# hip-satomi/microbeSEG

Hardware: AMD Instinct MI355X
Metric: training crops/sec (256px) (higher is better)
Workload: dtype f32; 1 GPU; BASELINE configs[1]: DU-Net distance-map training step, filters [64, 1024], 256x256 crops, per-GPU batch 32, fp32, relu/bn, SmoothL1x2 + Adam(amsgrad); global_batch=32, parallelism=dp1, launch=eager

## Files before the change

### include/mseg_hip.h

```cpp
#ifndef MSEG_HIP_H
#define MSEG_HIP_H

#include <stddef.h>
#include <stdint.h>

#ifdef __cplusplus
extern "C" {
#endif

#define MSEG_OK 0
#define MSEG_EINVAL (-1)
#define MSEG_ELAUNCH (-2)
#define MSEG_EWORKSPACE (-3)

#define MSEG_ACT_NONE 0
#define MSEG_ACT_RELU 1
#define MSEG_ACT_LEAKY 2
#define MSEG_ACT_ELU 3
#define MSEG_ACT_MISH 4

#define MSEG_NORM_BN 0
#define MSEG_NORM_GN 1
#define MSEG_NORM_IN 2

// ... 4 lines not shown
  const float* scale;
  const float* shift;
  int32_t C;
  int32_t act;
  int32_t ss;
  int32_t dtype;
} MsegSrc;

#define MSEG_MODE_CONV 0
#define MSEG_MODE_TCONV 1
#define MSEG_EPI_PLAIN 0
#define MSEG_EPI_SCATTER2X2 1
#define MSEG_MORDER_LINEAR 0
#define MSEG_MORDER_PARITY 1
#define MSEG_PREC_F32 0
#define MSEG_PREC_BF16 1

typedef struct MsegIgemm {
  MsegSrc src[2];
  const float* w;
  const float* bias;
  float* dst0;
  float* dst1;
  int32_t nsrc, Cin, Kpad, Npad;
  int32_t NB, Hi, Wi, Ho, Wo;
  int32_t KH, KW, stride, pad, mode, morder;
  int32_t Ngemm, epi, split, ld0, ld1, acc0, acc1, Cq;
  int32_t precision;
  int32_t dst_dtype;
  void* ws;
  size_t ws_bytes;
  float* stats;
  int32_t stats_act;
  int32_t reserved0;
} MsegIgemm;

int mseg_igemm(const MsegIgemm* p, void* stream);

typedef struct MsegKernelInfo {
  char name[120];
  int32_t precision;
  int32_t launches;
  uint32_t grid, block;
  size_t workspace;
  int32_t stats_rows;
  int32_t reserved0;
} MsegKernelInfo;
int mseg_igemm_query(const MsegIgemm* p, MsegKernelInfo* info);
const char* mseg_last_kernel(void);
int mseg_f32_to_bf16(const float* src, uint16_t* dst, size_t n, void* stream);
size_t mseg_igemm_workspace_bytes(const MsegIgemm* p);
int mseg_igemm_set_persistent(int on);
int mseg_igemm_set_wide_tiles(int on);
int mseg_igemm_set_p8(int mode);

typedef struct MsegWgrad {
  MsegSrc P;
  MsegSrc Q[2];
  float* ws;
  float* dst;
  int32_t nq, Nch, Nch_store;
  int32_t NB, Hp, Wp, Hq, Wq;
  int32_t KH, KW, stride, pad;
  int32_t splits;
  int32_t phase;
  int32_t precision;
  int32_t reserved;
// ... 288 lines not shown
```

### microbeseg_amd/_lib.py

```python
import ctypes as C
import os
import pathlib

_HERE = pathlib.Path(__file__).resolve().parent
LIB_PATH = _HERE / "libmseg_hip.so"

ACT = {"none": 0, "relu": 1, "leakyrelu": 2, "elu": 3, "mish": 4}
NORM = {"bn": 0, "gn": 1, "in": 2}
MODE_CONV, MODE_TCONV = 0, 1
EPI_PLAIN, EPI_SCATTER2X2 = 0, 1
MORDER_LINEAR, MORDER_PARITY = 0, 1
ST_F32, ST_BF16 = 0, 1
PIX_U8, PIX_U16, PIX_I32, PIX_F32 = 0, 1, 2, 3
GATHER_RAW, GATHER_F32, GATHER_NORM, GATHER_I64 = 0, 1, 2, 3


class MsegLibraryError(RuntimeError):
    pass


class MsegSrc(C.Structure):
    _fields_ = [("ptr", C.c_void_p), ("scale", C.c_void_p), ("shift", C.c_void_p),
                ("C", C.c_int32), ("act", C.c_int32), ("ss", C.c_int32), ("dtype", C.c_int32)]


class MsegIgemm(C.Structure):
    _fields_ = [("src", MsegSrc * 2), ("w", C.c_void_p), ("bias", C.c_void_p), ("dst0", C.c_void_p),
                ("dst1", C.c_void_p),
                ("nsrc", C.c_int32), ("Cin", C.c_int32), ("Kpad", C.c_int32), ("Npad", C.c_int32),
                ("NB", C.c_int32), ("Hi", C.c_int32), ("Wi", C.c_int32), ("Ho", C.c_int32), ("Wo", C.c_int32),
                ("KH", C.c_int32), ("KW", C.c_int32), ("stride", C.c_int32), ("pad", C.c_int32),
                ("mode", C.c_int32), ("morder", C.c_int32),
                ("Ngemm", C.c_int32), ("epi", C.c_int32), ("split", C.c_int32), ("ld0", C.c_int32),
                ("ld1", C.c_int32), ("acc0", C.c_int32), ("acc1", C.c_int32), ("Cq", C.c_int32),
                ("precision", C.c_int32), ("dst_dtype", C.c_int32), ("ws", C.c_void_p), ("ws_bytes", C.c_size_t),
                ("stats", C.c_void_p), ("stats_act", C.c_int32), ("reserved0", C.c_int32)]


class MsegWgrad(C.Structure):
    _fields_ = [("P", MsegSrc), ("Q", MsegSrc * 2), ("ws", C.c_void_p), ("dst", C.c_void_p),
                ("nq", C.c_int32), ("Nch", C.c_int32), ("Nch_store", C.c_int32),
                ("NB", C.c_int32), ("Hp", C.c_int32), ("Wp", C.c_int32), ("Hq", C.c_int32), ("Wq", C.c_int32),
                ("KH", C.c_int32), ("KW", C.c_int32), ("stride", C.c_int32), ("pad", C.c_int32),
                ("splits", C.c_int32), ("phase", C.c_int32), ("precision", C.c_int32), ("reserved", C.c_int32)]


class MsegKernelInfo(C.Structure):
    _fields_ = [("name", C.c_char * 120), ("precision", C.c_int32), ("launches", C.c_int32), ("grid", C.c_uint32),
                ("block", C.c_uint32), ("workspace", C.c_size_t), ("stats_rows", C.c_int32), ("reserved0", C.c_int32)]


class MsegPackJob(C.Structure):
    _fields_ = [("src", C.c_void_p), ("dst", C.c_void_p), ("dst16", C.c_void_p),
                ("T", C.c_int32), ("R", C.c_int32), ("Rpad", C.c_int32), ("C", C.c_int32), ("Cpad", C.c_int32),
                ("st", C.c_int32), ("sr", C.c_int32), ("sc", C.c_int32),
                ("first_block", C.c_uint32), ("reserved", C.c_uint32)]


class MsegRangerJob(C.Structure):
    _fields_ = [("p", C.c_void_p), ("g", C.c_void_p), ("m", C.c_void_p), ("v", C.c_void_p), ("slow", C.c_void_p),
                ("n", C.c_uint64), ("rows", C.c_int32), ("step_lr", C.c_float), ("flags", C.c_uint32),
                ("reserved", C.c_uint32)]


class MsegTtaMember(C.Structure):
    _fields_ = [("ptr", C.c_void_p), ("frame_stride", C.c_int64), ("chan_stride", C.c_int64), ("row_stride", C.c_int64),
                ("pix_stride", C.c_int64), ("code", C.c_int32), ("reserved", C.c_int32)]


# ... 180 lines not shown
```

### microbeseg_amd/csrc/igemm.hip

```cpp
#include "common.h"
#include "igemm_common.h"
#include "bf16_affine.h"

int igemm_p8_try(const MsegIgemm& p, int tr, int m_fastest, int cus, hipStream_t st);

__device__ float g_ident_scale[MSEG_MAX_CH];
__device__ float g_ident_shift[MSEG_MAX_CH];
__global__ void init_ident_kernel() {
  for (int i = blockIdx.x * blockDim.x + threadIdx.x; i < MSEG_MAX_CH; i += gridDim.x * blockDim.x) {
    g_ident_scale[i] = 1.f;
    g_ident_shift[i] = 0.f;
  }
}


template <int BM, int BN, bool PER_SAMPLE, bool GENERIC_ACT>
__global__ __launch_bounds__(256) void igemm_kernel(const MsegIgemm p) {
  using Cfg = IgemmCfg<BM, BN>;
  constexpr int STAGE = (BM + BN) * LDS_STRIDE;
  __shared__ __attribute__((aligned(16))) float lds[2 * STAGE + 4];
  unsigned* tapmask_s = reinterpret_cast<unsigned*>(lds + 2 * STAGE);

  const int tid = threadIdx.x;
  const int lane = tid & 63;
  const int wave = tid >> 6;
  const int wm = wave / Cfg::WN, wn = wave % Cfg::WN;

  const int M = p.NB * p.Ho * p.Wo;
  const int ntiles_n = (p.Ngemm + BN - 1) / BN;
  const int lid = (int)xcd_logical_id(blockIdx.x, gridDim.x);
  const int tile_m = lid / ntiles_n;
  const int tile_n = lid - tile_m * ntiles_n;
  const int m0 = tile_m * BM, n0 = tile_n * BN;

  const int T = p.KH * p.KW;
  const int srow = tid >> 3;
  const int scol = tid & 7;
// ... 170 lines not shown
        for (int b = 0; b < Cfg::NB; ++b) {
          acc[a][b] = __builtin_amdgcn_mfma_f32_32x32x2f32(af[a].x, bf[b].x, acc[a][b], 0, 0, 0);
          acc[a][b] = __builtin_amdgcn_mfma_f32_32x32x2f32(af[a].y, bf[b].y, acc[a][b], 0, 0, 0);
          acc[a][b] = __builtin_amdgcn_mfma_f32_32x32x2f32(af[a].z, bf[b].z, acc[a][b], 0, 0, 0);
          acc[a][b] = __builtin_amdgcn_mfma_f32_32x32x2f32(af[a].w, bf[b].w, acc[a][b], 0, 0, 0);
        }
    }
    float* An = lds + (cur ^ 1) * STAGE;
#ifdef MSEG_ABLATE
    STAMP(s2);
    if (!(abl & 8)) commit(An, An + BM * LDS_STRIDE);
    STAMP(s3);
    if (!(abl & 2)) __syncthreads();
    STAMP(s4);
    t_issue += s1 - s0; t_mfma += s2 - s1; t_commit += s3 - s2; t_bar += s4 - s3;
#else
    commit(An, An + BM * LDS_STRIDE);
    __syncthreads();
#endif
    cur ^= 1;
    have = have_next;
  }

#ifdef MSEG_ABLATE
  if ((abl & 32) && p.dst1 && lane == 0 && blockIdx.x < 1024) {
    float* dbg = p.dst1 + ((size_t)blockIdx.x * 4 + wave) * 4;
    dbg[0] = (float)t_issue; dbg[1] = (float)t_mfma; dbg[2] = (float)t_commit; dbg[3] = (float)t_bar;
  }
#endif
  igemm_epilogue<IgemmCfg<BM, BN>>(acc, m0, n0, wm, wn, lane, M);
}

template <int BM, int BN, int TR, bool PER_SAMPLE, bool SB = false>
__global__ __launch_bounds__(256) void igemm_fast_kernel(const MsegIgemm p) {
  using Cfg = IgemmCfg<BM, BN>;
  constexpr int STAGE = (BM + BN) * LDS_STRIDE;
  __shared__ __attribute__((aligned(16))) float lds[(SB ? 1 : 2) * STAGE];

  const int tid = threadIdx.x;
  const int lane = tid & 63;
  const int wave = tid >> 6;
  const int wm = wave / Cfg::WN, wn = wave % Cfg::WN;
  const int M = p.NB * p.Ho * p.Wo;
  const int ntiles_n = (p.Ngemm + BN - 1) / BN;
  const int lid = (int)xcd_logical_id(blockIdx.x, gridDim.x);
  const int tile_m = lid / ntiles_n;
  const int tile_n = lid - tile_m * ntiles_n;
  const int m0 = tile_m * BM, n0 = tile_n * BN;
  const int T = p.KH * p.KW;
  const int srow = tid >> 3, scol = tid & 7;

  const TapGeom geom = make_geom(p);
  const long long tile_px = tile_base_pixel(p, geom, m0, M);
  int pix0[Cfg::AROWS];
  int rown[Cfg::AROWS];
  unsigned vmask[Cfg::AROWS];
#pragma unroll
  for (int i = 0; i < Cfg::AROWS; ++i) {
    const RowInfo r = decode_row(p, m0 + srow + 32 * i, M);
    const int iy0 = (r.oy * geom.sm - geom.dir * geom.pad) >> geom.sh, ix0 = (r.ox * geom.sm - geom.dir * geom.pad) >> geom.sh;
    pix0[i] = (int)(((long long)r.n * p.Hi + iy0) * p.Wi + ix0 - tile_px);
    rown[i] = r.n < 0 ? 0 : r.n;
    unsigned mk = 0u;
    for (int t = 0; t < T; ++t) {
      const int ky = t / p.KW, kx = t - ky * p.KW;
      int iy, ix;
      mk |= (unsigned)tap_coord(geom, r, ky, kx, iy, ix) << t;
    }
    vmask[i] = mk;
  }

  f32x16 acc[Cfg::MB][Cfg::NB];
#pragma unroll
  for (int a = 0; a < Cfg::MB; ++a)
#pragma unroll
    for (int b = 0; b < Cfg::NB; ++b)
#pragma unroll
      for (int r = 0; r < 16; ++r) acc[a][b][r] = 0.f;

  const int nchunks = (p.Cin + KC - 1) / KC;
  const int C0 = p.src[0].C;
  const unsigned OOB = 0x80000000u;

  const __amdgpu_buffer_rsrc_t rs0 = __builtin_amdgcn_make_buffer_rsrc(
      const_cast<float*>(p.src[0].ptr + tile_px * p.src[0].C), 0, 0x7ffffff0, 0x00020000);
  const __amdgpu_buffer_rsrc_t rs1 = __builtin_amdgcn_make_buffer_rsrc(
      const_cast<float*>((p.nsrc > 1 ? p.src[1].ptr : p.src[0].ptr) + tile_px * (p.nsrc > 1 ? p.src[1].C : p.src[0].C)), 0,
      0x7ffffff0, 0x00020000);
  const __amdgpu_buffer_rsrc_t rsw = __builtin_amdgcn_make_buffer_rsrc(const_cast<float*>(p.w), 0,
                                                                        T * p.Npad * p.Kpad * 4, 0x00020000);
  unsigned wvoff[Cfg::BROWS];
#pragma unroll
  for (int i = 0; i < Cfg::BROWS; ++i) wvoff[i] = ((unsigned)(n0 + srow + 32 * i) * (unsigned)p.Kpad + scol * 4u) * 4u;

  constexpr int NSC = (TR == 0) ? 1 : (PER_SAMPLE ? Cfg::AROWS : 1);
  float4 ra[Cfg::AROWS], rb[Cfg::BROWS], rsc[NSC], rsh[NSC];
  float rm[Cfg::AROWS];
  unsigned rowoff[Cfg::AROWS];
  int ract = 0;
  int cur_chunk = -1;
  bool cur_s1 = false;

  auto issue = [&](int chunk, int t, int ky, int kx) {
    const int c = chunk * KC + scol * 4;
    if (chunk != cur_chunk) {
      cur_chunk = chunk;
      cur_s1 = (p.nsrc > 1) && (chunk * KC >= C0);
      const unsigned sC4 = (unsigned)(cur_s1 ? p.src[1].C : p.src[0].C) * 4u;
      const unsigned cl4 = (unsigned)(cur_s1 ? c - C0 : c) * 4u;
#pragma unroll
      for (int i = 0; i < Cfg::AROWS; ++i) rowoff[i] = (unsigned)pix0[i] * sC4 + cl4;
      if (TR != 0) {
        const MsegSrc& s = cur_s1 ? p.src[1] : p.src[0];
        ract = s.act;
        const bool has_aff = s.scale != nullptr;
        const float* scp = has_aff ? s.scale : g_ident_scale;
        const float* shp = has_aff ? s.shift : g_ident_shift;
        const unsigned cl = (c < p.Cin) ? (cl4 >> 2) : 0u;
#pragma unroll
        for (int i = 0; i < NSC; ++i) {
          const size_t o = (size_t)(PER_SAMPLE ? rown[i] : 0) * (has_aff ? (unsigned)s.ss : 0u) + cl;
          rsc[i] = *reinterpret_cast<const float4*>(scp + o);
          rsh[i] = *reinterpret_cast<const float4*>(shp + o);
        }
      }
    }
    const unsigned cbit = (c < p.Cin) ? (1u << t) : 0u;
    const unsigned sC4 = (unsigned)(cur_s1 ? p.src[1].C : p.src[0].C) * 4u;
    const unsigned delta = (unsigned)(geom.dir * ((ky >> geom.sh) * p.Wi + (kx >> geom.sh))) * sC4;
#pragma unroll
    for (int i = 0; i < Cfg::AROWS; ++i) {
      const bool ok = (vmask[i] & cbit) != 0u;
      const unsigned vo = ok ? rowoff[i] + delta : OOB;
// ... 3 lines not shown
      if (TR != 0) rm[i] = ok ? 1.f : 0.f;
    }
    const unsigned wso = ((unsigned)t * (unsigned)p.Npad * (unsigned)p.Kpad + (unsigned)chunk * KC) * 4u;
#pragma unroll
    for (int i = 0; i < Cfg::BROWS; ++i) {
      const f32x4 v = __builtin_bit_cast(f32x4, __builtin_amdgcn_raw_buffer_load_b128(rsw, wvoff[i], wso, 0));
      rb[i] = make_float4(v[0], v[1], v[2], v[3]);
    }
  };

  auto commit = [&](float* As, float* Bs) {
    const float lo = (ract == MSEG_ACT_RELU) ? 0.f : -3.402823466e38f;
#pragma unroll
    for (int i = 0; i < Cfg::AROWS; ++i) {
      float4 v = ra[i];
      if (TR != 0) {
        if (TR == 2) {
          v = act_fwd4(v, ract);
        } else {
          v.x = clamp_lo(v.x, lo); v.y = clamp_lo(v.y, lo); v.z = clamp_lo(v.z, lo); v.w = clamp_lo(v.w, lo);
        }
        const float4 sc = rsc[PER_SAMPLE ? i : 0], sh = rsh[PER_SAMPLE ? i : 0];
        const float m = rm[i];
        v.x = (v.x * sc.x + sh.x) * m; v.y = (v.y * sc.y + sh.y) * m;
        v.z = (v.z * sc.z + sh.z) * m; v.w = (v.w * sc.w + sh.w) * m;
      }
      *reinterpret_cast<float4*>(As + (srow + 32 * i) * LDS_STRIDE + scol * 4) = v;
    }
#pragma unroll
    for (int i = 0; i < Cfg::BROWS; ++i)
      *reinterpret_cast<float4*>(Bs + (srow + 32 * i) * LDS_STRIDE + scol * 4) = rb[i];
  };

  unsigned long long taplist = 0ull, taplist_hi = 0ull;
  int nlive = 0;
  {
    int py = 0, px = 0;
    if (geom.sh) {
      const int cls = m0 / (M >> 2);
      py = cls >> 1; px = cls & 1;
    }
    for (int tt = 0; tt < T; ++tt) {
      const int ky_ = tt / p.KW, kx_ = tt - ky_ * p.KW;
      const bool live = (((py - geom.dir * (ky_ - geom.pad)) | (px - geom.dir * (kx_ - geom.pad))) & geom.sh) == 0;
      if (live) {
        const unsigned long long e = (unsigned long long)(tt | (ky_ << 4) | (kx_ << 6));
        if (nlive < 8) taplist |= e << (8 * nlive); else taplist_hi |= e << (8 * (nlive - 8));
        ++nlive;
      }
    }
  }
  auto tap_at = [&](int j) -> unsigned { return (unsigned)((j < 8 ? taplist >> (8 * j) : taplist_hi >> (8 * (j - 8))) & 0xffull); };
  int chunk = 0, j = 0;
  const int nsteps = nchunks * nlive;
  unsigned e0 = tap_at(0);
  issue(0, (int)(e0 & 15u), (int)((e0 >> 4) & 3u), (int)(e0 >> 6));
  commit(lds, lds + BM * LDS_STRIDE);
  __syncthreads();
  int cur = 0;
  const int li = lane & 31, lh = lane >> 5;
  for (int step = 0; step < nsteps; ++step) {
    if (step + 1 < nsteps) {
      j += 1;
      if (j >= nlive) { j = 0; ++chunk; }
    }
    e0 = tap_at(j);
    issue(chunk, (int)(e0 & 15u), (int)((e0 >> 4) & 3u), (int)(e0 >> 6));

    const float* As = lds + cur * STAGE;
    const float* Bs = As + BM * LDS_STRIDE;
#pragma unroll
    for (int kk = 0; kk < KC / 8; ++kk) {
      float4 af[Cfg::MB], bf[Cfg::NB];
#pragma unroll
      for (int a = 0; a < Cfg::MB; ++a)
        af[a] = *reinterpret_cast<const float4*>(As + (wm * Cfg::TM + a * 32 + li) * LDS_STRIDE + kk * 8 + lh * 4);
#pragma unroll
      for (int b = 0; b < Cfg::NB; ++b)
        bf[b] = *reinterpret_cast<const float4*>(Bs + (wn * Cfg::TN + b * 32 + li) * LDS_STRIDE + kk * 8 + lh * 4);
#pragma unroll
      for (int a = 0; a < Cfg::MB; ++a)
#pragma unroll
        for (int b = 0; b < Cfg::NB; ++b) {
          acc[a][b] = __builtin_amdgcn_mfma_f32_32x32x2f32(af[a].x, bf[b].x, acc[a][b], 0, 0, 0);
          acc[a][b] = __builtin_amdgcn_mfma_f32_32x32x2f32(af[a].y, bf[b].y, acc[a][b], 0, 0, 0);
          acc[a][b] = __builtin_amdgcn_mfma_f32_32x32x2f32(af[a].z, bf[b].z, acc[a][b], 0, 0, 0);
          acc[a][b] = __builtin_amdgcn_mfma_f32_32x32x2f32(af[a].w, bf[b].w, acc[a][b], 0, 0, 0);
        }
    }
    if (SB) {
      __syncthreads();
      commit(lds, lds + BM * LDS_STRIDE);
      __syncthreads();
    } else {
      float* An = lds + (cur ^ 1) * STAGE;
      commit(An, An + BM * LDS_STRIDE);
      __syncthreads();
      cur ^= 1;
    }
  }
  igemm_epilogue<IgemmCfg<BM, BN>>(acc, m0, n0, wm, wn, lane, M);
}

template <int BN>
struct HaloCfg {
  static constexpr int WN = (BN >= 128) ? 4 : 2;
  static constexpr int WM = 8 / WN;
  static constexpr int TM = 128 / WM, TN = BN / WN;
  static constexpr int MB = TM / 32, NB = TN / 32;
  static constexpr int BROWS = BN / 64;
};

template <int BN, int TR>
__global__ __launch_bounds__(512, 2) void igemm_halo_kernel(const MsegIgemm p, int tw_log2, int ksplit,
                                                            int chunks_per_split) {
  constexpr int BM = 128;
  using Cfg = HaloCfg<BN>;
  constexpr int HMAX = 264;
  constexpr int HL = (HMAX * 8 + 511) / 512;
  constexpr int ASTAGE = HMAX * LDS_STRIDE;
  constexpr int BSTAGE = BN * LDS_STRIDE;
  __shared__ __attribute__((aligned(16))) float lds[ASTAGE + 2 * BSTAGE];
  float* const Abuf = lds;
  float* const Bbuf = lds + ASTAGE;

  const int tid = threadIdx.x, lane = tid & 63, wave = tid >> 6;
  const int wm = wave / Cfg::WN, wn = wave % Cfg::WN;
  const int li = lane & 31, lh = lane >> 5;
  const int srow = tid >> 3, scol = tid & 7;
  const int TW = 1 << tw_log2, TH = BM >> tw_log2, HW2 = TW + 2;
  const int HROWS = (TH + 2) * HW2;
  const int H = p.Hi, W = p.Wi;
  const int M = p.NB * H * W;
  const int tiles_x = W >> tw_log2, tiles_y = (H + TH - 1) / TH;
// ... 1957 lines not shown
}

extern "C" size_t mseg_igemm_workspace_bytes(const MsegIgemm* pp) {
  if (!pp) return 0;
  const MsegIgemm& p = *pp;
  if (p.Ngemm <= 0 || p.Cin <= 0 || p.NB <= 0 || p.Hi <= 0 || p.Wi <= 0) return 0;
  int tw_log2 = 0, cps = 0;
  long long htiles = 0;
  if (!halo_geometry(p, p.Ngemm > 64 ? 128 : 64, &tw_log2, &htiles)) return 0;
  const int ks = halo_ksplit(htiles, (p.Cin + KC - 1) / KC, &cps);
  if (ks <= 1 || (p.Ngemm & 3)) return 0;
  return (size_t)ks * p.NB * p.Hi * p.Wi * p.Ngemm * sizeof(float);
}

static int igemm_dispatch(const MsegIgemm* pp, void* stream) {
  if (!pp) return MSEG_EINVAL;
  const MsegIgemm& p = *pp;
  if (p.nsrc < 1 || p.nsrc > 2) return MSEG_EINVAL;
  int csum = 0;
  for (int i = 0; i < p.nsrc; ++i) {
    if (check_src(p.src[i])) return MSEG_EINVAL;
    csum += p.src[i].C;
  }
  if (csum != p.Cin) return MSEG_EINVAL;
  if (!p.w || !p.dst0 || p.Kpad < p.Cin || (p.Kpad % KC) || p.Npad < p.Ngemm || (p.Npad % 128)) return MSEG_EINVAL;
  if (p.Cin > MSEG_MAX_CH) return MSEG_EINVAL;
  if (p.NB <= 0 || p.Hi <= 0 || p.Wi <= 0 || p.Ho <= 0 || p.Wo <= 0) return MSEG_EINVAL;
  if (p.KH <= 0 || p.KW <= 0 || p.KH * p.KW > 16) return MSEG_EINVAL;
  if (p.stride != 1 && p.stride != 2) return MSEG_EINVAL;
  if (p.mode != MSEG_MODE_CONV && p.mode != MSEG_MODE_TCONV) return MSEG_EINVAL;
  if (p.morder == MSEG_MORDER_PARITY && ((p.Ho | p.Wo) & 1)) return MSEG_EINVAL;
  if (p.Ngemm <= 0) return MSEG_EINVAL;
  if (p.precision != MSEG_PREC_F32 && p.precision != MSEG_PREC_BF16) return MSEG_EINVAL;
  if (p.dst_dtype != MSEG_ST_F32 && p.dst_dtype != MSEG_ST_BF16) return MSEG_EINVAL;
  const bool s16 = p.src[0].dtype == MSEG_ST_BF16;
  if (p.nsrc > 1 && p.src[1].dtype != p.src[0].dtype) return MSEG_EINVAL;
  if ((s16 || p.dst_dtype == MSEG_ST_BF16) && p.precision != MSEG_PREC_BF16) return MSEG_EINVAL;
  if (p.dst_dtype == MSEG_ST_BF16) {
    if ((p.Ngemm | p.ld0 | p.ld1 | p.Cq) & 1) return MSEG_EINVAL;
    if (p.split < p.Ngemm && (p.split & 1)) return MSEG_EINVAL;
    if (((uintptr_t)p.dst0 | (uintptr_t)p.dst1) & 3) return MSEG_EINVAL;
  }
  if (p.epi == MSEG_EPI_SCATTER2X2) {
    if (p.Cq <= 0 || p.Ngemm != 4 * p.Cq || p.morder != MSEG_MORDER_LINEAR) return MSEG_EINVAL;
  } else if (p.epi == MSEG_EPI_PLAIN) {
    if (p.split < p.Ngemm && !p.dst1) return MSEG_EINVAL;
  } else {
    return MSEG_EINVAL;
  }
  const long long M = (long long)p.NB * p.Ho * p.Wo;
  if (M <= 0 || M > 0x7fffffffLL) return MSEG_EINVAL;
  hipStream_t st = (hipStream_t)stream;
  mseg_dispatch_note(p.precision, 0);
  static bool ident_ready[64] = {false};
  int devid = 0;
  const bool dry = mseg_dispatch_dry() != 0;
  if (!dry) {
    if (hipGetDevice(&devid) != hipSuccess || devid < 0 || devid >= 64) return MSEG_ELAUNCH;
    if (!ident_ready[devid]) {
      MSEG_KL_AUX(init_ident_kernel, dim3(8), dim3(256), 0, st);
      MSEG_LAUNCH_CHECK();
      ident_ready[devid] = true;
    }
  }
  bool per_sample = false, generic = false;
  for (int i = 0; i < p.nsrc; ++i) {
// ... 139 lines not shown
      p.stride == 2 && p.pad == 0 && p.mode == MSEG_MODE_CONV && p.morder == MSEG_MORDER_LINEAR && p.nsrc == 1 &&
      p.Cin == 64 && p.Kpad == 64 && p.Ngemm == 128 && p.split >= p.Ngemm && !p.acc0 && !p.bias && (p.Wo % 32) == 0 &&
      p.Hi == 2 * p.Ho && p.Wi == 2 * p.Wo && (M % 64) == 0 && M / 64 >= 4 * (long long)c64p_workgroups()) {
    const dim3 pgrid((unsigned)c64p_workgroups());
    if (p.dst_dtype == MSEG_ST_BF16) MSEG_KL((igemm_ctd_bf16_kernel<true>), pgrid, dim3(512), 0, st, p, (int)(M / 64));
    else MSEG_KL((igemm_ctd_bf16_kernel<false>), pgrid, dim3(512), 0, st, p, (int)(M / 64));
    MSEG_LAUNCH_CHECK();
    return MSEG_OK;
  }
  if (p.precision == MSEG_PREC_BF16) {
    if (!fast) return MSEG_EINVAL;
    const int tr = plain ? 0 : (generic ? 2 : 1);
#define MSEG_FAST16_LAUNCH(BM_, BN_, TR_, PS_)                                                          \
  do {                                                                                                  \
    if (s16) MSEG_KL((igemm_fast_bf16_kernel<BM_, BN_, TR_, PS_, true>), grid, block, 0, st, p);   \
    else MSEG_KL((igemm_fast_bf16_kernel<BM_, BN_, TR_, PS_, false>), grid, block, 0, st, p);      \
  } while (0)
#define MSEG_FAST16_TILE(BM_, BN_)                                                        \
  do {                                                                                    \
    if (tr == 0) MSEG_FAST16_LAUNCH(BM_, BN_, 0, false);                                  \
    else if (tr == 1) { if (per_sample) MSEG_FAST16_LAUNCH(BM_, BN_, 1, true); else MSEG_FAST16_LAUNCH(BM_, BN_, 1, false); } \
    else { if (per_sample) MSEG_FAST16_LAUNCH(BM_, BN_, 2, true); else MSEG_FAST16_LAUNCH(BM_, BN_, 2, false); }              \
  } while (0)
    if (wide) MSEG_FAST16_TILE(128, 128); else MSEG_FAST16_TILE(128, 64);
#undef MSEG_FAST16_TILE
#undef MSEG_FAST16_LAUNCH
    MSEG_LAUNCH_CHECK();
    return MSEG_OK;
  }
  if (fast) {
    const int tr = plain ? 0 : (generic ? 2 : 1);
    const int live_taps = (p.mode == MSEG_MODE_TCONV && p.stride == 2) ? ((p.KH + 1) / 2) * ((p.KW + 1) / 2) : p.KH * p.KW;
    const bool short_k = ((p.Cin + KC - 1) / KC) * live_taps <= 8;
#define MSEG_FAST_LAUNCH(BM_, BN_, TR_, PS_)                                                              \
  do {                                                                                                    \
    if (short_k) MSEG_KL((igemm_fast_kernel<BM_, BN_, TR_, PS_, true>), grid, block, 0, st, p); \
    else MSEG_KL((igemm_fast_kernel<BM_, BN_, TR_, PS_, false>), grid, block, 0, st, p);        \
  } while (0)
#define MSEG_FAST_TILE(BM_, BN_)                                                          \
  do {                                                                                    \
    if (tr == 0) MSEG_FAST_LAUNCH(BM_, BN_, 0, false);                                    \
    else if (tr == 1) { if (per_sample) MSEG_FAST_LAUNCH(BM_, BN_, 1, true); else MSEG_FAST_LAUNCH(BM_, BN_, 1, false); } \
    else { if (per_sample) MSEG_FAST_LAUNCH(BM_, BN_, 2, true); else MSEG_FAST_LAUNCH(BM_, BN_, 2, false); }              \
  } while (0)
    if (wide) MSEG_FAST_TILE(128, 128); else MSEG_FAST_TILE(128, 64);
#undef MSEG_FAST_TILE
#undef MSEG_FAST_LAUNCH
    MSEG_LAUNCH_CHECK();
    return MSEG_OK;
  }
#define MSEG_IGEMM_LAUNCH(BM_, BN_, PS_, GA_) \
  MSEG_KL((igemm_kernel<BM_, BN_, PS_, GA_>), grid, block, 0, st, p)
  if (wide) {
    if (per_sample) { if (generic) MSEG_IGEMM_LAUNCH(128, 128, true, true); else MSEG_IGEMM_LAUNCH(128, 128, true, false); }
    else            { if (generic) MSEG_IGEMM_LAUNCH(128, 128, false, true); else MSEG_IGEMM_LAUNCH(128, 128, false, false); }
  } else {
    if (per_sample) { if (generic) MSEG_IGEMM_LAUNCH(128, 64, true, true); else MSEG_IGEMM_LAUNCH(128, 64, true, false); }
    else            { if (generic) MSEG_IGEMM_LAUNCH(128, 64, false, true); else MSEG_IGEMM_LAUNCH(128, 64, false, false); }
  }
#undef MSEG_IGEMM_LAUNCH
  MSEG_LAUNCH_CHECK();
  return MSEG_OK;
}

extern "C" int mseg_igemm(const MsegIgemm* pp, void* stream) {
  mseg_dispatch_begin(0);
  const int rc = igemm_dispatch(pp, stream);
  mseg_dispatch_end(nullptr);
  return rc;
}
// ... 100 lines not shown
```

Measured before the change: 243.8 crops/s.

## Make fp32 fast implicit-GEMM kernel persistent over multiple M tiles per workgroup

The fp32 fast implicit-GEMM kernel now loops over several M tiles per workgroup in a serpentine order, with the grid sized from CU count and occupancy. The next tile's row geometry and tap list are set up during the last K step of the current tile, and per-row geometry is staged through shared memory. Launch bounds now request two or three workgroups per CU. This aims to cut tail-wave waste and per-block setup cost, at the price of more register and LDS pressure and extra control flow in the main loop.

```diff
diff --git a/include/mseg_hip.h b/include/mseg_hip.h
--- a/include/mseg_hip.h
+++ b/include/mseg_hip.h
@@ -60,7 +60,7 @@
   size_t ws_bytes;
   float* stats;
   int32_t stats_act;
-  int32_t reserved0;
+  int32_t tiles_per_wg;
 } MsegIgemm;
 
 int mseg_igemm(const MsegIgemm* p, void* stream);
diff --git a/microbeseg_amd/_lib.py b/microbeseg_amd/_lib.py
--- a/microbeseg_amd/_lib.py
+++ b/microbeseg_amd/_lib.py
@@ -34,7 +34,7 @@
                 ("Ngemm", C.c_int32), ("epi", C.c_int32), ("split", C.c_int32), ("ld0", C.c_int32),
                 ("ld1", C.c_int32), ("acc0", C.c_int32), ("acc1", C.c_int32), ("Cq", C.c_int32),
                 ("precision", C.c_int32), ("dst_dtype", C.c_int32), ("ws", C.c_void_p), ("ws_bytes", C.c_size_t),
-                ("stats", C.c_void_p), ("stats_act", C.c_int32), ("reserved0", C.c_int32)]
+                ("stats", C.c_void_p), ("stats_act", C.c_int32), ("tiles_per_wg", C.c_int32)]
 
 
 class MsegWgrad(C.Structure):
diff --git a/microbeseg_amd/csrc/igemm.hip b/microbeseg_amd/csrc/igemm.hip
--- a/microbeseg_amd/csrc/igemm.hip
+++ b/microbeseg_amd/csrc/igemm.hip
@@ -239,10 +239,11 @@
 }
 
 template <int BM, int BN, int TR, bool PER_SAMPLE, bool SB = false>
-__global__ __launch_bounds__(256) void igemm_fast_kernel(const MsegIgemm p) {
+__global__ __launch_bounds__(256, (BN == 64 && SB && TR == 0) ? 3 : 2) void igemm_fast_kernel(const MsegIgemm p) {
   using Cfg = IgemmCfg<BM, BN>;
   constexpr int STAGE = (BM + BN) * LDS_STRIDE;
   __shared__ __attribute__((aligned(16))) float lds[(SB ? 1 : 2) * STAGE];
+  __shared__ int geo[3 * BM];
 
   const int tid = threadIdx.x;
   const int lane = tid & 63;
@@ -250,62 +251,93 @@
   const int wm = wave / Cfg::WN, wn = wave % Cfg::WN;
   const int M = p.NB * p.Ho * p.Wo;
   const int ntiles_n = (p.Ngemm + BN - 1) / BN;
+  const int mtiles = (M + BM - 1) / BM;
   const int lid = (int)xcd_logical_id(blockIdx.x, gridDim.x);
-  const int tile_m = lid / ntiles_n;
-  const int tile_n = lid - tile_m * ntiles_n;
-  const int m0 = tile_m * BM, n0 = tile_n * BN;
+  const int G = (int)gridDim.x / ntiles_n;
+  const int grp = lid / ntiles_n;
+  const int tile_n = lid - grp * ntiles_n;
+  const int n0 = tile_n * BN;
+  if (grp >= mtiles) return;
   const int T = p.KH * p.KW;
-  const int srow = tid >> 3, scol = tid & 7;
+  int srow = tid >> 3, scol = tid & 7;
 
   const TapGeom geom = make_geom(p);
-  const long long tile_px = tile_base_pixel(p, geom, m0, M);
   int pix0[Cfg::AROWS];
   int rown[Cfg::AROWS];
   unsigned vmask[Cfg::AROWS];
-#pragma unroll
-  for (int i = 0; i < Cfg::AROWS; ++i) {
-    const RowInfo r = decode_row(p, m0 + srow + 32 * i, M);
-    const int iy0 = (r.oy * geom.sm - geom.dir * geom.pad) >> geom.sh, ix0 = (r.ox * geom.sm - geom.dir * geom.pad) >> geom.sh;
-    pix0[i] = (int)(((long long)r.n * p.Hi + iy0) * p.Wi + ix0 - tile_px);
-    rown[i] = r.n < 0 ? 0 : r.n;
-    unsigned mk = 0u;
-    for (int t = 0; t < T; ++t) {
-      const int ky = t / p.KW, kx = t - ky * p.KW;
-      int iy, ix;
-      mk |= (unsigned)tap_coord(geom, r, ky, kx, iy, ix) << t;
-    }
-    vmask[i] = mk;
-  }
+  __amdgpu_buffer_rsrc_t rs0, rs1;
+  unsigned long long taplist = 0ull, taplist_hi = 0ull;
+  int nlive = 0;
+  int cur_chunk = -1;
+
+  auto setup = [&](int m0) {
+    const long long tile_px = tile_base_pixel(p, geom, m0, M);
+#pragma unroll
+    for (int i = 0; i < Cfg::AROWS; ++i) {
+      const RowInfo r = decode_row(p, m0 + srow + 32 * i, M);
+      const int iy0 = (r.oy * geom.sm - geom.dir * geom.pad) >> geom.sh, ix0 = (r.ox * geom.sm - geom.dir * geom.pad) >> geom.sh;
+      pix0[i] = (int)(((long long)r.n * p.Hi + iy0) * p.Wi + ix0 - tile_px);
+      rown[i] = r.n < 0 ? 0 : r.n;
+      unsigned ym = 0u, xm = 0u;
+      for (int k = 0; k < p.KH; ++k) {
+        const int ty = r.oy * geom.sm + geom.dir * (k - geom.pad), iy = ty >> geom.sh;
+        ym |= (unsigned)(((ty & geom.sh) == 0) & (iy >= 0) & (iy < geom.Hi)) << k;
+      }
+      for (int k = 0; k < p.KW; ++k) {
+        const int tx = r.ox * geom.sm + geom.dir * (k - geom.pad), ix = tx >> geom.sh;
+        xm |= (unsigned)(((tx & geom.sh) == 0) & (ix >= 0) & (ix < geom.Wi)) << k;
+      }
+      if (r.n < 0) ym = 0u;
+      unsigned mk = 0u;
+      for (int ky = 0; ky < p.KH; ++ky) mk |= (((ym >> ky) & 1u) ? xm : 0u) << (ky * p.KW);
+      vmask[i] = mk;
+      const int gr = srow + 32 * i;
+      geo[gr] = pix0[i]; geo[BM + gr] = (int)mk; geo[2 * BM + gr] = rown[i];
+    }
+    rs0 = __builtin_amdgcn_make_buffer_rsrc(const_cast<float*>(p.src[0].ptr + tile_px * p.src[0].C), 0, 0x7ffffff0,
+                                            0x00020000);
+    rs1 = __builtin_amdgcn_make_buffer_rsrc(
+        const_cast<float*>((p.nsrc > 1 ? p.src[1].ptr : p.src[0].ptr) + tile_px * (p.nsrc > 1 ? p.src[1].C : p.src[0].C)), 0,
+        0x7ffffff0, 0x00020000);
+    int py = 0, px = 0;
+    if (geom.sh) {
+      const int cls = m0 / (M >> 2);
+      py = cls >> 1; px = cls & 1;
+    }
+    taplist = 0ull; taplist_hi = 0ull; nlive = 0;
+    int tt = 0;
+    for (int ky_ = 0; ky_ < p.KH; ++ky_)
+      for (int kx_ = 0; kx_ < p.KW; ++kx_, ++tt) {
+        const bool live = (((py - geom.dir * (ky_ - geom.pad)) | (px - geom.dir * (kx_ - geom.pad))) & geom.sh) == 0;
+        if (live) {
+          const unsigned long long e = (unsigned long long)(tt | (ky_ << 4) | (kx_ << 6));
+          if (nlive < 8) taplist |= e << (8 * nlive); else taplist_hi |= e << (8 * (nlive - 8));
+          ++nlive;
+        }
+      }
+    cur_chunk = -1;
+  };
 
   f32x16 acc[Cfg::MB][Cfg::NB];
-#pragma unroll
-  for (int a = 0; a < Cfg::MB; ++a)
-#pragma unroll
-    for (int b = 0; b < Cfg::NB; ++b)
-#pragma unroll
-      for (int r = 0; r < 16; ++r) acc[a][b][r] = 0.f;
 
   const int nchunks = (p.Cin + KC - 1) / KC;
   const int C0 = p.src[0].C;
   const unsigned OOB = 0x80000000u;
 
-  const __amdgpu_buffer_rsrc_t rs0 = __builtin_amdgcn_make_buffer_rsrc(
-      const_cast<float*>(p.src[0].ptr + tile_px * p.src[0].C), 0, 0x7ffffff0, 0x00020000);
-  const __amdgpu_buffer_rsrc_t rs1 = __builtin_amdgcn_make_buffer_rsrc(
-      const_cast<float*>((p.nsrc > 1 ? p.src[1].ptr : p.src[0].ptr) + tile_px * (p.nsrc > 1 ? p.src[1].C : p.src[0].C)), 0,
-      0x7ffffff0, 0x00020000);
   const __amdgpu_buffer_rsrc_t rsw = __builtin_amdgcn_make_buffer_rsrc(const_cast<float*>(p.w), 0,
                                                                         T * p.Npad * p.Kpad * 4, 0x00020000);
   unsigned wvoff[Cfg::BROWS];
-#pragma unroll
-  for (int i = 0; i < Cfg::BROWS; ++i) wvoff[i] = ((unsigned)(n0 + srow + 32 * i) * (unsigned)p.Kpad + scol * 4u) * 4u;
+  auto set_wvoff = [&]() {
+#pragma unroll
+    for (int i = 0; i < Cfg::BROWS; ++i) wvoff[i] = ((unsigned)(n0 + srow + 32 * i) * (unsigned)p.Kpad + scol * 4u) * 4u;
+  };
+  set_wvoff();
 
   constexpr int NSC = (TR == 0) ? 1 : (PER_SAMPLE ? Cfg::AROWS : 1);
   float4 ra[Cfg::AROWS], rb[Cfg::BROWS], rsc[NSC], rsh[NSC];
   float rm[Cfg::AROWS];
   unsigned rowoff[Cfg::AROWS];
   int ract = 0;
-  int cur_chunk = -1;
   bool cur_s1 = false;
 
   auto issue = [&](int chunk, int t, int ky, int kx) {
@@ -375,74 +407,89 @@
       *reinterpret_cast<float4*>(Bs + (srow + 32 * i) * LDS_STRIDE + scol * 4) = rb[i];
   };
 
-  unsigned long long taplist = 0ull, taplist_hi = 0ull;
-  int nlive = 0;
-  {
-    int py = 0, px = 0;
-    if (geom.sh) {
-      const int cls = m0 / (M >> 2);
-      py = cls >> 1; px = cls & 1;
-    }
-    for (int tt = 0; tt < T; ++tt) {
-      const int ky_ = tt / p.KW, kx_ = tt - ky_ * p.KW;
-      const bool live = (((py - geom.dir * (ky_ - geom.pad)) | (px - geom.dir * (kx_ - geom.pad))) & geom.sh) == 0;
-      if (live) {
-        const unsigned long long e = (unsigned long long)(tt | (ky_ << 4) | (kx_ << 6));
-        if (nlive < 8) taplist |= e << (8 * nlive); else taplist_hi |= e << (8 * (nlive - 8));
-        ++nlive;
-      }
-    }
-  }
   auto tap_at = [&](int j) -> unsigned { return (unsigned)((j < 8 ? taplist >> (8 * j) : taplist_hi >> (8 * (j - 8))) & 0xffull); };
+  int tile_m = grp, blk = 0;
+  setup(tile_m * BM);
   int chunk = 0, j = 0;
-  const int nsteps = nchunks * nlive;
+  int nsteps = nchunks * nlive;
   unsigned e0 = tap_at(0);
   issue(0, (int)(e0 & 15u), (int)((e0 >> 4) & 3u), (int)(e0 >> 6));
   commit(lds, lds + BM * LDS_STRIDE);
   __syncthreads();
   int cur = 0;
-  const int li = lane & 31, lh = lane >> 5;
-  for (int step = 0; step < nsteps; ++step) {
-    if (step + 1 < nsteps) {
-      j += 1;
-      if (j >= nlive) { j = 0; ++chunk; }
-    }
-    e0 = tap_at(j);
-    issue(chunk, (int)(e0 & 15u), (int)((e0 >> 4) & 3u), (int)(e0 >> 6));
-
-    const float* As = lds + cur * STAGE;
-    const float* Bs = As + BM * LDS_STRIDE;
-#pragma unroll
-    for (int kk = 0; kk < KC / 8; ++kk) {
-      float4 af[Cfg::MB], bf[Cfg::NB];
-#pragma unroll
-      for (int a = 0; a < Cfg::MB; ++a)
-        af[a] = *reinterpret_cast<const float4*>(As + (wm * Cfg::TM + a * 32 + li) * LDS_STRIDE + kk * 8 + lh * 4);
+  int li = lane & 31, lh = lane >> 5;
+  for (;;) {
+    const int m0 = tile_m * BM;
+    const int nblk = blk + 1;
+    const int next_m = nblk * G + ((nblk & 1) ? G - 1 - grp : grp);
+    const bool more = next_m < mtiles;
+    int nsteps_next = 0;
+#pragma unroll
+    for (int a = 0; a < Cfg::MB; ++a)
 #pragma unroll
       for (int b = 0; b < Cfg::NB; ++b)
-        bf[b] = *reinterpret_cast<const float4*>(Bs + (wn * Cfg::TN + b * 32 + li) * LDS_STRIDE + kk * 8 + lh * 4);
-#pragma unroll
-      for (int a = 0; a < Cfg::MB; ++a)
-#pragma unroll
-        for (int b = 0; b < Cfg::NB; ++b) {
-          acc[a][b] = __builtin_amdgcn_mfma_f32_32x32x2f32(af[a].x, bf[b].x, acc[a][b], 0, 0, 0);
-          acc[a][b] = __builtin_amdgcn_mfma_f32_32x32x2f32(af[a].y, bf[b].y, acc[a][b], 0, 0, 0);
-          acc[a][b] = __builtin_amdgcn_mfma_f32_32x32x2f32(af[a].z, bf[b].z, acc[a][b], 0, 0, 0);
-          acc[a][b] = __builtin_amdgcn_mfma_f32_32x32x2f32(af[a].w, bf[b].w, acc[a][b], 0, 0, 0);
-        }
-    }
-    if (SB) {
-      __syncthreads();
-      commit(lds, lds + BM * LDS_STRIDE);
-      __syncthreads();
-    } else {
-      float* An = lds + (cur ^ 1) * STAGE;
-      commit(An, An + BM * LDS_STRIDE);
-      __syncthreads();
-      cur ^= 1;
-    }
-  }
-  igemm_epilogue<IgemmCfg<BM, BN>>(acc, m0, n0, wm, wn, lane, M);
+#pragma unroll
+        for (int r = 0; r < 16; ++r) acc[a][b][r] = 0.f;
+    for (int step = 0; step < nsteps; ++step) {
+      if (step + 1 < nsteps) {
+        j += 1;
+        if (j >= nlive) { j = 0; ++chunk; }
+      } else if (more) {
+        setup(next_m * BM);
+        nsteps_next = nchunks * nlive;
+        chunk = 0; j = 0;
+      }
+      e0 = tap_at(j);
+      issue(chunk, (int)(e0 & 15u), (int)((e0 >> 4) & 3u), (int)(e0 >> 6));
+
+      const float* As = lds + cur * STAGE;
+      const float* Bs = As + BM * LDS_STRIDE;
+#pragma unroll
+      for (int kk = 0; kk < KC / 8; ++kk) {
+        float4 af[Cfg::MB], bf[Cfg::NB];
+#pragma unroll
+        for (int a = 0; a < Cfg::MB; ++a)
+          af[a] = *reinterpret_cast<const float4*>(As + (wm * Cfg::TM + a * 32 + li) * LDS_STRIDE + kk * 8 + lh * 4);
+#pragma unroll
+        for (int b = 0; b < Cfg::NB; ++b)
+          bf[b] = *reinterpret_cast<const float4*>(Bs + (wn * Cfg::TN + b * 32 + li) * LDS_STRIDE + kk * 8 + lh * 4);
+#pragma unroll
+        for (int a = 0; a < Cfg::MB; ++a)
+#pragma unroll
+          for (int b = 0; b < Cfg::NB; ++b) {
+            acc[a][b] = __builtin_amdgcn_mfma_f32_32x32x2f32(af[a].x, bf[b].x, acc[a][b], 0, 0, 0);
+            acc[a][b] = __builtin_amdgcn_mfma_f32_32x32x2f32(af[a].y, bf[b].y, acc[a][b], 0, 0, 0);
+            acc[a][b] = __builtin_amdgcn_mfma_f32_32x32x2f32(af[a].z, bf[b].z, acc[a][b], 0, 0, 0);
+            acc[a][b] = __builtin_amdgcn_mfma_f32_32x32x2f32(af[a].w, bf[b].w, acc[a][b], 0, 0, 0);
+          }
+      }
+      if (SB) {
+        __syncthreads();
+        commit(lds, lds + BM * LDS_STRIDE);
+        __syncthreads();
+      } else {
+        float* An = lds + (cur ^ 1) * STAGE;
+        commit(An, An + BM * LDS_STRIDE);
+        __syncthreads();
+        cur ^= 1;
+      }
+    }
+    igemm_epilogue<IgemmCfg<BM, BN>>(acc, m0, n0, wm, wn, lane, M);
+    if (!more) break;
+    tile_m = next_m;
+    blk = nblk;
+    int t_ = tid;
+    asm volatile("" : "+v"(t_));
+    srow = t_ >> 3; scol = t_ & 7; li = t_ & 31; lh = (t_ >> 5) & 1;
+#pragma unroll
+    for (int i = 0; i < Cfg::AROWS; ++i) {
+      const int gr = srow + 32 * i;
+      pix0[i] = geo[gr]; vmask[i] = (unsigned)geo[BM + gr]; rown[i] = geo[2 * BM + gr];
+    }
+    set_wvoff();
+    cur_chunk = -1;
+    nsteps = nsteps_next;
+  }
 }
 
 template <int BN>
@@ -2466,6 +2513,7 @@
   if (p.morder == MSEG_MORDER_PARITY && ((p.Ho | p.Wo) & 1)) return MSEG_EINVAL;
   if (p.Ngemm <= 0) return MSEG_EINVAL;
   if (p.precision != MSEG_PREC_F32 && p.precision != MSEG_PREC_BF16) return MSEG_EINVAL;
+  if (p.tiles_per_wg < 0 || p.tiles_per_wg > 64) return MSEG_EINVAL;
   if (p.dst_dtype != MSEG_ST_F32 && p.dst_dtype != MSEG_ST_BF16) return MSEG_EINVAL;
   const bool s16 = p.src[0].dtype == MSEG_ST_BF16;
   if (p.nsrc > 1 && p.src[1].dtype != p.src[0].dtype) return MSEG_EINVAL;
@@ -2671,10 +2719,22 @@
     const int tr = plain ? 0 : (generic ? 2 : 1);
     const int live_taps = (p.mode == MSEG_MODE_TCONV && p.stride == 2) ? ((p.KH + 1) / 2) * ((p.KW + 1) / 2) : p.KH * p.KW;
     const bool short_k = ((p.Cin + KC - 1) / KC) * live_taps <= 8;
+    const long long mtiles = (M + BMv - 1) / BMv, ntn = (p.Ngemm + BNv - 1) / BNv;
+    long long tpw = p.tiles_per_wg;
+    if (tpw == 0) {
+      tpw = 1;
+      const long long slots = (long long)c64p_workgroups() * ((short_k && !wide && tr == 0) ? 3 : 2);
+      if (tiles > slots && p.morder != MSEG_MORDER_PARITY) tpw = 2;
+      else if (tiles > slots) {
+        const long long rounds = ((tiles + slots - 1) / slots + 15) / 16;
+        for (tpw = 2; tpw < 64 && ((mtiles + tpw - 1) / tpw) * ntn > slots * rounds; ++tpw) {}
+      }
+    }
+    const dim3 fgrid((unsigned)(((mtiles + tpw - 1) / tpw) * ntn));
 #define MSEG_FAST_LAUNCH(BM_, BN_, TR_, PS_)                                                              \
   do {                                                                                                    \
-    if (short_k) MSEG_KL((igemm_fast_kernel<BM_, BN_, TR_, PS_, true>), grid, block, 0, st, p); \
-    else MSEG_KL((igemm_fast_kernel<BM_, BN_, TR_, PS_, false>), grid, block, 0, st, p);        \
+    if (short_k) MSEG_KL((igemm_fast_kernel<BM_, BN_, TR_, PS_, true>), fgrid, block, 0, st, p); \
+    else MSEG_KL((igemm_fast_kernel<BM_, BN_, TR_, PS_, false>), fgrid, block, 0, st, p);        \
   } while (0)
 #define MSEG_FAST_TILE(BM_, BN_)                                                          \
   do {                                                                                    \
```

Result: no change. 244.1 crops/s (median of 2 runs) (+0.1%).

## Add dense 512-thread igemm kernel for 1x1 scatter and 2x2 stride-2 convs

Applied to the files above, without the earlier changes.

Adds a specialized implicit-GEMM kernel for dense cases: the 1x1 transposed-conv forward with 2x2 scatter epilogue and the 2x2 stride-2 conv (its gradient counterpart). It uses 128x128 tiles, 8 waves, buffer loads with precomputed row offsets and magic-number division, and f32 MFMA. The aim is to skip generic tap and mask handling and get more reuse per tile. The cost is one more kernel to maintain, a single LDS buffer with two barriers per step, and strict eligibility checks, so shapes that fail them fall back to the existing path.

```diff
diff --git a/microbeseg_amd/csrc/igemm.hip b/microbeseg_amd/csrc/igemm.hip
--- a/microbeseg_amd/csrc/igemm.hip
+++ b/microbeseg_amd/csrc/igemm.hip
@@ -3,6 +3,7 @@
 #include "bf16_affine.h"
 
 int igemm_p8_try(const MsegIgemm& p, int tr, int m_fastest, int cus, hipStream_t st);
+int igemm_dense_try(const MsegIgemm& p, int tr, bool per_sample, int cus, hipStream_t st);
 
 __device__ float g_ident_scale[MSEG_MAX_CH];
 __device__ float g_ident_shift[MSEG_MAX_CH];
@@ -2671,6 +2672,8 @@
     const int tr = plain ? 0 : (generic ? 2 : 1);
     const int live_taps = (p.mode == MSEG_MODE_TCONV && p.stride == 2) ? ((p.KH + 1) / 2) * ((p.KW + 1) / 2) : p.KH * p.KW;
     const bool short_k = ((p.Cin + KC - 1) / KC) * live_taps <= 8;
+    const int drc = igemm_dense_try(p, tr, per_sample, c64p_workgroups(), st);
+    if (drc != 0) return drc < 0 ? drc : MSEG_OK;
 #define MSEG_FAST_LAUNCH(BM_, BN_, TR_, PS_)                                                              \
   do {                                                                                                    \
     if (short_k) MSEG_KL((igemm_fast_kernel<BM_, BN_, TR_, PS_, true>), grid, block, 0, st, p); \
diff --git a/microbeseg_amd/csrc/igemm_dense.hip b/microbeseg_amd/csrc/igemm_dense.hip
--- /dev/null
+++ b/microbeseg_amd/csrc/igemm_dense.hip
@@ -0,0 +1,186 @@
+#include "igemm_common.h"
+
+struct DenseCfg {
+  static constexpr int BM = 128, BN = 128;
+  static constexpr int WM = 2, WN = 4;
+  static constexpr int TM = BM / WM, TN = BN / WN;
+  static constexpr int MB = TM / 32, NB = TN / 32;
+  static constexpr int AROWS = BM / 64, BROWS = BN / 64;
+};
+
+template <int TR, bool T4>
+__global__ __launch_bounds__(512, 4) void igemm_dense_kernel(const MsegIgemm p, unsigned magic_w, unsigned magic_h) {
+  using Cfg = DenseCfg;
+  constexpr int BM = Cfg::BM, BN = Cfg::BN;
+  __shared__ __attribute__((aligned(16))) float lds[(BM + BN) * LDS_STRIDE];
+  float* const As = lds;
+  float* const Bs = lds + BM * LDS_STRIDE;
+
+  const int tid = threadIdx.x, lane = tid & 63, wave = tid >> 6;
+  const int wm = wave / Cfg::WN, wn = wave % Cfg::WN;
+  const int li = lane & 31, lh = lane >> 5;
+  const int srow = tid >> 3, scol = tid & 7;
+  const int M = p.NB * p.Ho * p.Wo;
+  const int ntiles_n = (p.Ngemm + BN - 1) / BN;
+  const int lid = (int)xcd_logical_id(blockIdx.x, gridDim.x);
+  const int tile_m = lid / ntiles_n, tile_n = lid - tile_m * ntiles_n;
+  const int m0 = tile_m * BM, n0 = tile_n * BN;
+  const int C = p.src[0].C;
+
+  long long tile_px;
+  unsigned rowoff[Cfg::AROWS];
+  if (!T4) {
+    tile_px = m0;
+#pragma unroll
+    for (int i = 0; i < Cfg::AROWS; ++i) rowoff[i] = (unsigned)(srow + 64 * i) * (unsigned)C * 4u + scol * 16u;
+  } else {
+    const int HoWo = p.Ho * p.Wo;
+    const int img0 = m0 / HoWo;
+    const int rem0 = m0 - img0 * HoWo;
+    const int by = rem0 / p.Wo, bx = rem0 - by * p.Wo;
+    tile_px = ((long long)img0 * p.Hi + 2 * by) * p.Wi + 2 * bx;
+#pragma unroll
+    for (int i = 0; i < Cfg::AROWS; ++i) {
+      int x = bx + srow + 64 * i;
+      const int dy = (int)__umulhi((unsigned)x, magic_w);
+      x -= dy * p.Wo;
+      int y = by + dy;
+      const int dn = (int)__umulhi((unsigned)y, magic_h);
+      y -= dn * p.Ho;
+      const int rel = (dn * p.Hi + 2 * (y - by)) * p.Wi + 2 * (x - bx);
+      rowoff[i] = (unsigned)rel * (unsigned)C * 4u + scol * 16u;
+    }
+  }
+
+  f32x16 acc[Cfg::MB][Cfg::NB];
+#pragma unroll
+  for (int a = 0; a < Cfg::MB; ++a)
+#pragma unroll
+    for (int b = 0; b < Cfg::NB; ++b)
+#pragma unroll
+      for (int r = 0; r < 16; ++r) acc[a][b][r] = 0.f;
+
+  constexpr int T = T4 ? 4 : 1;
+  const long long src_left = ((long long)p.NB * p.Hi * p.Wi - tile_px) * C * 4;
+  const __amdgpu_buffer_rsrc_t rsa = __builtin_amdgcn_make_buffer_rsrc(
+      const_cast<float*>(p.src[0].ptr + tile_px * C), 0, (int)(src_left < 0x7ffffff0LL ? src_left : 0x7ffffff0LL), 0x00020000);
+  const __amdgpu_buffer_rsrc_t rsw = __builtin_amdgcn_make_buffer_rsrc(const_cast<float*>(p.w), 0,
+                                                                        T * p.Npad * p.Kpad * 4, 0x00020000);
+  unsigned wvoff[Cfg::BROWS];
+#pragma unroll
+  for (int i = 0; i < Cfg::BROWS; ++i) wvoff[i] = ((unsigned)(n0 + srow + 64 * i) * (unsigned)p.Kpad + scol * 4u) * 4u;
+
+  float4 ra[Cfg::AROWS], rb[Cfg::BROWS];
+  float4 rsc = make_float4(1.f, 1.f, 1.f, 1.f), rsh = make_float4(0.f, 0.f, 0.f, 0.f);
+  const int ract = p.src[0].act;
+  const bool has_aff = p.src[0].scale != nullptr;
+
+  auto issue = [&](int chunk, int t) {
+    const unsigned aso = ((unsigned)chunk * KC + (unsigned)((t >> 1) * p.Wi + (t & 1)) * (unsigned)C) * 4u;
+#pragma unroll
+    for (int i = 0; i < Cfg::AROWS; ++i) {
+      const f32x4 v = __builtin_bit_cast(f32x4, __builtin_amdgcn_raw_buffer_load_b128(rsa, rowoff[i], aso, 0));
+      ra[i] = make_float4(v[0], v[1], v[2], v[3]);
+    }
+    const unsigned wso = ((unsigned)t * (unsigned)p.Npad * (unsigned)p.Kpad + (unsigned)chunk * KC) * 4u;
+#pragma unroll
+    for (int i = 0; i < Cfg::BROWS; ++i) {
+      const f32x4 v = __builtin_bit_cast(f32x4, __builtin_amdgcn_raw_buffer_load_b128(rsw, wvoff[i], wso, 0));
+      rb[i] = make_float4(v[0], v[1], v[2], v[3]);
+    }
+    if (TR != 0 && t == 0 && has_aff) {
+      rsc = *reinterpret_cast<const float4*>(p.src[0].scale + chunk * KC + scol * 4);
+      rsh = *reinterpret_cast<const float4*>(p.src[0].shift + chunk * KC + scol * 4);
+    }
+  };
+
+  auto commit = [&]() {
+    const float lo = (ract == MSEG_ACT_RELU) ? 0.f : -3.402823466e38f;
+#pragma unroll
+    for (int i = 0; i < Cfg::AROWS; ++i) {
+      float4 v = ra[i];
+      if (TR != 0) {
+        v.x = clamp_lo(v.x, lo); v.y = clamp_lo(v.y, lo); v.z = clamp_lo(v.z, lo); v.w = clamp_lo(v.w, lo);
+        v.x = v.x * rsc.x + rsh.x; v.y = v.y * rsc.y + rsh.y;
+        v.z = v.z * rsc.z + rsh.z; v.w = v.w * rsc.w + rsh.w;
+      }
+      *reinterpret_cast<float4*>(As + (srow + 64 * i) * LDS_STRIDE + scol * 4) = v;
+    }
+#pragma unroll
+    for (int i = 0; i < Cfg::BROWS; ++i)
+      *reinterpret_cast<float4*>(Bs + (srow + 64 * i) * LDS_STRIDE + scol * 4) = rb[i];
+  };
+
+  const int nsteps = (p.Cin / KC) * T;
+  issue(0, 0);
+  commit();
+  __syncthreads();
+  int chunk = 0, t = 0;
+  for (int step = 0; step < nsteps; ++step) {
+    const bool more = step + 1 < nsteps;
+    if (more) {
+      if (++t >= T) { t = 0; ++chunk; }
+      issue(chunk, t);
+    }
+#pragma unroll
+    for (int kk = 0; kk < KC / 8; ++kk) {
+      float4 af[Cfg::MB], bf[Cfg::NB];
+#pragma unroll
+      for (int a = 0; a < Cfg::MB; ++a)
+        af[a] = *reinterpret_cast<const float4*>(As + (wm * Cfg::TM + a * 32 + li) * LDS_STRIDE + kk * 8 + lh * 4);
+#pragma unroll
+      for (int b = 0; b < Cfg::NB; ++b)
+        bf[b] = *reinterpret_cast<const float4*>(Bs + (wn * Cfg::TN + b * 32 + li) * LDS_STRIDE + kk * 8 + lh * 4);
+#pragma unroll
+      for (int a = 0; a < Cfg::MB; ++a)
+#pragma unroll
+        for (int b = 0; b < Cfg::NB; ++b) {
+          acc[a][b] = __builtin_amdgcn_mfma_f32_32x32x2f32(af[a].x, bf[b].x, acc[a][b], 0, 0, 0);
+          acc[a][b] = __builtin_amdgcn_mfma_f32_32x32x2f32(af[a].y, bf[b].y, acc[a][b], 0, 0, 0);
+          acc[a][b] = __builtin_amdgcn_mfma_f32_32x32x2f32(af[a].z, bf[b].z, acc[a][b], 0, 0, 0);
+          acc[a][b] = __builtin_amdgcn_mfma_f32_32x32x2f32(af[a].w, bf[b].w, acc[a][b], 0, 0, 0);
+        }
+    }
+    if (more) {
+      __syncthreads();
+      commit();
+      __syncthreads();
+    }
+  }
+  igemm_epilogue<Cfg>(acc, m0, n0, wm, wn, lane, M);
+}
+
+int igemm_dense_try(const MsegIgemm& p, int tr, bool per_sample, int cus, hipStream_t st) {
+  if (p.precision != MSEG_PREC_F32 || p.dst_dtype != MSEG_ST_F32 || p.src[0].dtype != MSEG_ST_F32) return 0;
+  if (p.nsrc != 1 || tr > 1 || per_sample) return 0;
+  if ((p.Cin % KC) != 0 || p.Cin < 64 || p.Ngemm < 128) return 0;
+  if (p.mode != MSEG_MODE_CONV || p.morder != MSEG_MORDER_LINEAR) return 0;
+  const bool fwd = p.epi == MSEG_EPI_SCATTER2X2 && p.KH == 1 && p.KW == 1 && p.stride == 1 && p.pad == 0 &&
+                   p.Hi == p.Ho && p.Wi == p.Wo;
+  const bool dgr = p.epi == MSEG_EPI_PLAIN && p.KH == 2 && p.KW == 2 && p.stride == 2 && p.pad == 0 &&
+                   p.Hi == 2 * p.Ho && p.Wi == 2 * p.Wo;
+  if (!fwd && !dgr) return 0;
+  const long long M = (long long)p.NB * p.Ho * p.Wo;
+  if (M % DenseCfg::BM) return 0;
+  const long long tiles = (M / DenseCfg::BM) * ((p.Ngemm + DenseCfg::BN - 1) / DenseCfg::BN);
+  if (tiles < 2LL * cus || tiles > 0x7fffffffLL) return 0;
+  unsigned magic_w = 0, magic_h = 0;
+  if (dgr) {
+    if (p.Ho < 2 || p.Wo < 2 || p.Ho > 32768 || p.Wo > 32768) return 0;
+    magic_w = (unsigned)((1ULL << 32) / (unsigned)p.Wo) + 1u;
+    magic_h = (unsigned)((1ULL << 32) / (unsigned)p.Ho) + 1u;
+    if ((2LL * (128 / p.Wo + 3) + 2) * p.Wi * p.src[0].C * 4 >= 0x7ffffff0LL) return 0;
+  } else if (129LL * p.src[0].C * 4 >= 0x7ffffff0LL) {
+    return 0;
+  }
+  const dim3 grid((unsigned)tiles), block(512);
+  if (dgr) {
+    if (tr == 0) MSEG_KL((igemm_dense_kernel<0, true>), grid, block, 0, st, p, magic_w, magic_h);
+    else MSEG_KL((igemm_dense_kernel<1, true>), grid, block, 0, st, p, magic_w, magic_h);
+  } else {
+    if (tr == 0) MSEG_KL((igemm_dense_kernel<0, false>), grid, block, 0, st, p, magic_w, magic_h);
+    else MSEG_KL((igemm_dense_kernel<1, false>), grid, block, 0, st, p, magic_w, magic_h);
+  }
+  MSEG_LAUNCH_CHECK();
+  return 1;
+}
```

Measured after the change: 244.6 crops/s before, 245.8 crops/s after, median of 6. No clear change (+0.5%).
